# ibharvey/speq

Measured on AMD Instinct MI355X. Metric: k-mers scanned/sec (whole node) at k=21, 150 bp reads, higher is better.
Workload: dtype u32; 1 GPU; BASELINE config 2: 10 variants x 1 isolates x 50000 bp, 1000000 x 150 bp reads per GPU, k=21, global; k=21, reads_per_gpu=1000000, paired=False, mode=global, parallelism=dp1 (reads sharded, index replicated), collective=none (one GPU), gpus_visible=1, ranks_per_gpu=1, index_builder=gpu, fm_text_len=1000021

## Files before the change

### include/speq_scan.h

```cpp
#ifndef SPEQ_SCAN_H
#define SPEQ_SCAN_H

#include <stddef.h>
#include <stdint.h>

#ifdef __cplusplus
extern "C" {
#endif

#define SPEQ_ABI_VERSION 8

enum {
    SPEQ_OK = 0,
    SPEQ_E_ARG = -1,
    SPEQ_E_IO = -2,
    SPEQ_E_DEVICE = -3,
    SPEQ_E_GROUPS = -4,
    SPEQ_E_NOMEM = -5,
    SPEQ_E_RETRY = -6
};

enum { SPEQ_MODE_GLOBAL = 0, SPEQ_MODE_LOCAL = 1 };

typedef struct speq_index speq_index;
// ... 5 lines not shown
    uint32_t pair_steps;
    uint32_t label_table;
    uint32_t gpu_build;
    int32_t device;
    uint32_t triple_steps;
} speq_build_opts;

typedef struct {
    uint32_t k;
    uint32_t phred_cutoff;
    uint32_t paired;
    uint32_t mode;
} speq_scan_params;

#define SPEQ_COUNTS_LEN(G) ((size_t)(G) + 2u)

const char* speq_last_error(void);
int speq_abi_version(void);
int speq_device_count(void);

int speq_index_build(const char* seq, const uint64_t* rec_offsets, uint32_t n_records,
                     const int32_t* group_of_rec, uint32_t n_group_entries, uint32_t n_groups,
                     const speq_build_opts* opts, speq_index** out);
int speq_index_save(const speq_index* idx, const char* path, const void* user_header, uint64_t header_len);
int speq_index_load(const char* path, speq_index** out, void** user_header, uint64_t* header_len);
int speq_index_read_header(const char* path, void** user_header, uint64_t* header_len);
void speq_index_free(speq_index* idx);
void speq_free(void* p);

typedef struct {
    uint64_t n;
    uint32_t n_texts;
    uint32_t n_records;
    uint32_t n_groups;
    uint32_t prefix_q;
    uint32_t pair_steps;
    uint32_t label_table;
    uint64_t n_runs;
    uint64_t device_bytes;
    uint32_t triple_steps;
} speq_index_info;
int speq_index_get_info(const speq_index* idx, speq_index_info* info);

int speq_index_array(const speq_index* idx, const char* name, const void** ptr, uint64_t* bytes);

int speq_device_warmup(int device, uint32_t streams);
int speq_device_open(const speq_index* idx, int device, speq_device_index** out);
int speq_device_close(speq_device_index* d);

int speq_scan_reads_device(speq_device_index* d, const uint8_t* d_seq, const uint8_t* d_qual,
                           const uint64_t* d_offsets, uint64_t n_reads, const speq_scan_params* params,
                           uint64_t* d_counts, double* d_weights, void* stream);

#define SPEQ_AX_STATS_N 40
int speq_scan_reads_device_stats(speq_device_index* d, const uint8_t* d_seq, const uint8_t* d_qual,
                                 const uint64_t* d_offsets, uint64_t n_reads, const speq_scan_params* params,
                                 uint64_t* d_counts, double* d_weights, uint64_t* stats);

int speq_scan_reads(speq_device_index* d, const uint8_t* seq, const uint8_t* qual, const uint64_t* offsets,
                    uint64_t n_reads, const speq_scan_params* params, uint64_t* counts, double* weights);

#define SPEQ_REPORT_MAX_K 1024
typedef struct {
    uint32_t passing;
    uint32_t unique;
    uint32_t shared;
    uint32_t first_group;
} speq_read_report;
#define SPEQ_SET_WORDS(G) (((size_t)(G) + 63u) / 64u)
int speq_report_reads_device(speq_device_index* d, const uint8_t* d_seq, const uint8_t* d_qual,
                             const uint64_t* d_offsets, uint64_t n_reads, const speq_scan_params* params,
                             speq_read_report* d_reports, uint64_t* d_sets, void* stream);
int speq_report_reads(speq_device_index* d, const uint8_t* seq, const uint8_t* qual, const uint64_t* offsets,
                      uint64_t n_reads, const speq_scan_params* params, speq_read_report* reports, uint64_t* sets);
#define SPEQ_MARKER_BINS 8
typedef struct {
    uint64_t markers, observed, hits, max_depth, depth_hist[SPEQ_MARKER_BINS];
} speq_marker_cov;
typedef struct speq_markers speq_markers;
int speq_markers_create(speq_device_index* d, const speq_scan_params* params, speq_markers** out);
int speq_markers_add_reads_device(speq_markers* m, const uint8_t* d_seq, const uint8_t* d_qual,
                                  const uint64_t* d_offsets, uint64_t n_reads, void* stream);
int speq_markers_add_reads(speq_markers* m, const uint8_t* seq, const uint8_t* qual, const uint64_t* offsets,
                           uint64_t n_reads);
int speq_markers_finalize(speq_markers* m, speq_marker_cov* out);
int speq_markers_list(speq_markers* m, uint64_t* n_markers, uint32_t* lo, uint32_t* group, uint32_t* depth);
void speq_markers_free(speq_markers* m);

#define SPEQ_BOOTSTRAP_MAX_REPLICATES 1024
typedef struct speq_bootstrap speq_bootstrap;
int speq_bootstrap_create(speq_device_index* d, const speq_scan_params* params, uint32_t replicates, uint64_t seed,
                          speq_bootstrap** out);
int speq_bootstrap_add_reads_device(speq_bootstrap* b, const uint8_t* d_seq, const uint8_t* d_qual,
                                    const uint64_t* d_offsets, uint64_t n_reads, uint64_t first_unit, void* stream);
int speq_bootstrap_add_reads(speq_bootstrap* b, const uint8_t* seq, const uint8_t* qual, const uint64_t* offsets,
                             uint64_t n_reads, uint64_t first_unit);
int speq_bootstrap_finalize(speq_bootstrap* b, uint64_t* counts, double* weights);
int speq_bootstrap_info(const speq_bootstrap* b, uint32_t* replicates, uint32_t* lds_path, uint64_t* units_added);
void speq_bootstrap_free(speq_bootstrap* b);
uint32_t speq_bootstrap_weight(uint64_t seed, uint64_t unit, uint32_t replicate);
typedef struct { double estimate, mean, se, lo, hi; uint64_t used; } speq_bootstrap_ci;
int speq_bootstrap_summary(const uint64_t* counts, const double* weights, uint32_t replicates, uint32_t n_groups,
                           const uint64_t* u_ref, const uint64_t* tot_ref, double unique_scale, double level,
                           speq_bootstrap_ci* out );
int speq_bootstrap_summary_percent(const double* percent, const double* estimate, const uint8_t* used_mask,
                                   uint32_t replicates, uint32_t n_groups, double level,
                                   speq_bootstrap_ci* out );
// ... 168 lines not shown
```

### speq_amd/api.py

```python
from __future__ import annotations

import ctypes as C
from dataclasses import dataclass
from typing import Optional, Sequence

import numpy as np

from ._lib import (MARKER_BINS, SPEQ_MODE_GLOBAL, SPEQ_MODE_LOCAL, BootstrapCI, BuildOpts, IndexInfo,
                   DedupStatsRecord, ScanParams, Slot, SpeqError, StreamStats, check, lib)

__all__ = ["FmIndex", "DeviceIndex", "Node", "Pipeline", "ScanResult", "ReadReport", "Markers", "MarkerCoverage", "Bootstrap",
           "Dedup", "DedupStats", "dedup_fingerprint", "bootstrap_summary", "bootstrap_summary_percent", "em_rows_step", "em_rows_refine", "Groupings", "EmHistogram", "Comm", "file_to_map", "unique_to_percent",
           "em_refine", "pack_records", "SpeqError", "SPEQ_MODE_GLOBAL", "SPEQ_MODE_LOCAL"]


def _u64p(a: np.ndarray):
    return a.ctypes.data_as(C.POINTER(C.c_uint64))


def pack_records(records: Sequence[bytes | str]) -> tuple[bytes, np.ndarray]:
    bs = [r.encode() if isinstance(r, str) else bytes(r) for r in records]
    off = np.zeros(len(bs) + 1, dtype=np.uint64)
    if bs:
        off[1:] = np.cumsum([len(b) for b in bs], dtype=np.uint64)
# ... 259 lines not shown
                  phred_cutoff: int = 30, paired: bool = False, local: bool = False, first_unit: int = 0):
        b = Bootstrap(self, k, replicates, seed, phred_cutoff, paired, local)
        try:
            b.add(seq, qual, offsets, first_unit)
            return b.finalize()
        finally:
            b.close()

    def bootstrap_fastq(self, path1: str, path2: Optional[str] = None, k: int = 21, replicates: int = 200,
                        seed: int = 1, phred_cutoff: int = 30, local: bool = False, threads: int = 4):
        G = self.n_groups
        counts = np.zeros((replicates + 1, G + 2), dtype=np.uint64)
        w = np.zeros((replicates + 1, G), dtype=np.float64) if local else None
        p = ScanParams(k, phred_cutoff, int(path2 is not None), SPEQ_MODE_LOCAL if local else SPEQ_MODE_GLOBAL)
        check(lib().speq_bootstrap_fastq(self._h, path1.encode(), path2.encode() if path2 else None, C.byref(p),
                                         replicates, seed, threads, _u64p(counts),
                                         w.ctypes.data_as(C.POINTER(C.c_double)) if w is not None else None, None))
        return counts, w

    def bootstrap_em_fastq(self, em: "EmHistogram", path1: str, path2: Optional[str] = None, k: int = 21,
                           replicates: int = 200, seed: int = 1, phred_cutoff: int = 30, local: bool = False,
                           threads: int = 4):
        G = self.n_groups
        counts = np.zeros((replicates + 1, G + 2), dtype=np.uint64)
        w = np.zeros((replicates + 1, G), dtype=np.float64) if local else None
        mult = np.zeros((replicates + 1, em.n_rows()), dtype=np.uint64)
        missed = C.c_uint64()
        p = ScanParams(k, phred_cutoff, int(path2 is not None), SPEQ_MODE_LOCAL if local else SPEQ_MODE_GLOBAL)
        check(lib().speq_bootstrap_em_fastq(self._h, em._h, path1.encode(), path2.encode() if path2 else None,
                                            C.byref(p), replicates, seed, threads, _u64p(counts),
                                            w.ctypes.data_as(C.POINTER(C.c_double)) if w is not None else None,
                                            _u64p(mult), C.byref(missed), None))
        return counts, w, mult, missed.value

    def dedup_fastq(self, path1: str, path2: Optional[str] = None, k: int = 21, phred_cutoff: int = 30,
                    local: bool = False, threads: int = 4, em: Optional["EmHistogram"] = None):
        G = self.n_groups
        counts = np.zeros(G + 2, dtype=np.uint64)
        w = np.zeros(G, dtype=np.float64) if local else None
        p = ScanParams(k, phred_cutoff, int(path2 is not None), SPEQ_MODE_LOCAL if local else SPEQ_MODE_GLOBAL)
        r = DedupStatsRecord()
        check(lib().speq_dedup_fastq(self._h, em._h if em is not None else None, path1.encode(),
                                     path2.encode() if path2 else None, C.byref(p), threads, C.byref(r),
                                     _u64p(counts), w.ctypes.data_as(C.POINTER(C.c_double)) if w is not None else None,
                                     None))
        return DedupStats.from_record(r), ScanResult(int(counts[0]), int(counts[1]), counts[2:].copy(), w)

    AX_STATS_KEYS = ("wave_iters", "lookup_lanes", "run_lanes", "lookup_waves", "run_waves", "run_windows",
                     "deferred", "filter_pass", "p2_probes", "p2_verify", "chunks", "segments", "qual_bytes",
                     "run_tallied", "run_granules", "refills", "busy_1_4", "busy_5_16", "busy_17_32", "busy_33_64",
                     "cyc_refill", "cyc_lookup", "cyc_run", "cyc_phase2", "cyc_total", "p2_passes",
                     "cyc_p2_filter", "p2_rounds", "cyc_ref_pre", "cyc_ref_stage", "cyc_wave_max", "waves",
                     "cyc_gen0", "cyc_gen1", "cyc_gen2", "cyc_gen3", "cyc_gen4",
                     "sproof_probes", "sproof_windows", "sproof_partial")

    def scan_device_stats(self, d_seq: int, d_qual: int, d_offsets: int, n_reads: int, k: int, d_counts: int,
                          d_weights: int = 0, phred_cutoff: int = 30, paired: bool = False,
                          local: bool = False) -> dict:
        p = ScanParams(k, phred_cutoff, int(paired), SPEQ_MODE_LOCAL if local else SPEQ_MODE_GLOBAL)
        st = np.zeros(len(self.AX_STATS_KEYS), dtype=np.uint64)
        check(lib().speq_scan_reads_device_stats(self._h, d_seq, d_qual, d_offsets, n_reads, C.byref(p), d_counts,
                                                 d_weights or None, _u64p(st)))
        return {key: int(v) for key, v in zip(self.AX_STATS_KEYS, st)}

    def scan_fastq(self, path1: str, path2: Optional[str] = None, k: int = 21, phred_cutoff: int = 30,
                   local: bool = False, threads: int = 4, em: Optional["EmHistogram"] = None):
        G = self.n_groups
        counts = np.zeros(G + 2, dtype=np.uint64)
        w = np.zeros(G, dtype=np.float64) if local else None
        p = ScanParams(k, phred_cutoff, int(path2 is not None), SPEQ_MODE_LOCAL if local else SPEQ_MODE_GLOBAL)
        st = StreamStats()
        check(lib().speq_scan_fastq(self._h, path1.encode(), path2.encode() if path2 else None, C.byref(p),
                                    em._h if em is not None else None, threads, _u64p(counts),
                                    w.ctypes.data_as(C.POINTER(C.c_double)) if w is not None else None,
                                    C.byref(st)))
        stats = {"records": st.records, "bases": st.bases, "batches": st.batches, "seconds": st.seconds}
        return ScanResult(int(counts[0]), int(counts[1]), counts[2:].copy(), w), stats

    def scan_fastq_shard(self, path1: str, path2: Optional[str], k: int, shard: int, n_shards: int, cut: int = 0,
                         phred_cutoff: int = 30, local: bool = False, threads: int = 4,
                         em: Optional["EmHistogram"] = None):
        G = self.n_groups
        counts = np.zeros(G + 2, dtype=np.uint64)
        w = np.zeros(G, dtype=np.float64) if local else None
        p = ScanParams(k, phred_cutoff, int(path2 is not None), SPEQ_MODE_LOCAL if local else SPEQ_MODE_GLOBAL)
        st = StreamStats()
        check(lib().speq_scan_fastq_shard(self._h, em._h if em is not None else None, path1.encode(),
                                          path2.encode() if path2 else None, C.byref(p), threads, shard, n_shards,
                                          cut, _u64p(counts),
                                          w.ctypes.data_as(C.POINTER(C.c_double)) if w is not None else None,
                                          C.byref(st)))
        stats = {"records": st.records, "bases": st.bases, "batches": st.batches, "seconds": st.seconds}
        return ScanResult(int(counts[0]), int(counts[1]), counts[2:].copy(), w), stats

    def count_unique_kmers_per_group_shard(self, k: int, shard: int, n_shards: int):
        G = self.n_groups
        u = np.zeros(G, dtype=np.uint64)
        t = np.zeros(G, dtype=np.uint64)
        check(lib().speq_ref_unique_shard(self._h, k, shard, n_shards, _u64p(u), _u64p(t)))
        return u, t

    def count_unique_kmers_per_group(self, k: int) -> tuple[np.ndarray, np.ndarray]:
        G = self.n_groups
        u = np.zeros(G, dtype=np.uint64)
        t = np.zeros(G, dtype=np.uint64)
        check(lib().speq_ref_unique(self._h, k, _u64p(u), _u64p(t)))
        return u, t
# ... 572 lines not shown
```

### speq_amd/csrc/ax_common.hpp

```cpp
#pragma once
#include <hip/hip_runtime.h>

#include <cstdint>

#include "scan_device.hpp"
#include "speq_scan.h"

namespace speq_dev {
struct AxView {
    const u32x4* gran;
    const uint32_t* mlo;
    const uint32_t* mhi;
    const unsigned long long* atab;
    const unsigned long long* filt;
    unsigned long long* stats;
    uint64_t nb;
    uint64_t nf;
    uint64_t n;
    uint64_t gran_bytes;
    uint64_t nmf;
    uint32_t mf_off;
    uint32_t m;
    uint32_t mtiles;
    uint32_t s_off;
    uint32_t s_bytes;
    uint32_t G;
};
}

namespace {

using namespace speq_dev;

constexpr uint32_t AX_MAX_K = 128;
constexpr uint32_t AX_CAP = 192;
constexpr uint32_t AX_STREAM = AX_CAP + 16;
constexpr uint32_t AX_CHUNKS = AX_STREAM / 16;
constexpr uint32_t AX_CMP = 160;
constexpr uint32_t AX_CMPW = AX_CMP / 32;
constexpr uint32_t AX_NGR = AX_CMPW + 1;
constexpr uint32_t AX_CHK = 3;
constexpr uint32_t AX_VWW = 4;
#ifndef SPEQ_AX_DEF_LOCAL
#define SPEQ_AX_DEF_LOCAL 416
#endif
#ifndef SPEQ_AX_DEF_GLOBAL
#define SPEQ_AX_DEF_GLOBAL 864
#endif
template <int MODE>
constexpr uint32_t ax_def() {
    return MODE == KM_LOCAL ? SPEQ_AX_DEF_LOCAL : SPEQ_AX_DEF_GLOBAL;
}
static_assert(SPEQ_AX_DEF_GLOBAL % 4 == 0 && SPEQ_AX_DEF_LOCAL % 4 == 0, "u64 counters after the deferred list");
constexpr uint32_t AX_F = 4;
constexpr uint32_t AX_EMPTY = 0xFFFFFFFFu;
constexpr uint16_t AX_VOID = 0xFFFFu;
constexpr unsigned long long AX_SLOT_EMPTY = ~0ull;
constexpr uint32_t AX_OOB = 0xFFFFFFF0u;
constexpr uint32_t AX_FILTER_BITS = 16;
constexpr uint32_t AX_MP = 4;
constexpr uint32_t AX_MAX_G = 0xFFFFu;
typedef unsigned int u32x2 __attribute__((ext_vector_type(2)));

enum : uint32_t { AX_OWN = 0, AX_MULTI = 1, AX_SENT = 2, AX_END = 3 };

static_assert(AX_STREAM % 16 == 0, "chunks of 16 bases");
static_assert(AX_CAP < 1024, "deferred entries hold the window in 10 bits");
static_assert(AX_CMP % 32 == 0 && AX_CMP <= AX_CAP && 64 * AX_CHK >= AX_CMP, "run geometry");

enum : uint32_t {
    AXS_WAVE_ITERS = 0,
    AXS_LOOKUP_LANES,
    AXS_RUN_LANES,
    AXS_LOOKUP_WAVES,
    AXS_RUN_WAVES,
    AXS_RUN_WINDOWS,
    AXS_DEFERRED,
    AXS_FILTER_PASS,
    AXS_P2_PROBES,
    AXS_P2_VERIFY,
    AXS_CHUNKS,
    AXS_SEGMENTS,
    AXS_QBYTES,
    AXS_RUN_TALLIED,
    AXS_RUN_GRANULES,
    AXS_REFILLS,
    AXS_BUSY_1_4,
    AXS_BUSY_5_16,
    AXS_BUSY_17_32,
    AXS_BUSY_33_64,
    AXS_CYC_REFILL,
    AXS_CYC_LOOKUP,
    AXS_CYC_RUN,
    AXS_CYC_P2,
    AXS_CYC_TOTAL,
    AXS_P2_PASSES,
    AXS_CYC_P2_FILTER,
    AXS_P2_ROUNDS,
    AXS_CYC_REF_PRE,
    AXS_CYC_REF_STAGE,
    AXS_CYC_WAVE_MAX,
    AXS_WAVES,
    AXS_CYC_GEN0,
    AXS_CYC_GEN1,
    AXS_CYC_GEN2,
    AXS_CYC_GEN3,
    AXS_CYC_GEN4,
    AXS_SPROOF_PROBES,
    AXS_SPROOF_WINDOWS,
    AXS_SPROOF_PARTIAL,
    AXS_N
};
static_assert(AXS_N == SPEQ_AX_STATS_N, "speq_scan.h SPEQ_AX_STATS_N");

__host__ __device__ __forceinline__ uint64_t ax_fmix(uint64_t x) {
    x ^= x >> 33;
    x *= 0xFF51AFD7ED558CCDull;
    x ^= x >> 33;
    x *= 0xC4CEB9FE1A85EC53ull;
    x ^= x >> 33;
    return x;
}

template <int NW>
__device__ __forceinline__ uint64_t ax_hash(const uint64_t (&w)[NW], uint32_t k) {
    uint64_t h = 0x9E3779B97F4A7C15ull * (uint64_t)(k + 1u);
#pragma unroll
    for (int i = 0; i < NW; ++i) {
        if (32u * (uint32_t)i < k) {
            const uint32_t rem = k - 32u * (uint32_t)i;
            uint64_t x = w[i];
            if (rem < 32u) x &= (1ull << (2u * rem)) - 1ull;
            h = ax_fmix(h ^ x);
        }
    }
    return h;
}
__host__ __device__ __forceinline__ uint32_t ax_bucket(uint64_t h, uint64_t nb) {
    return (uint32_t)(((h >> 32) * nb) >> 32);
}
__host__ __device__ __forceinline__ uint32_t ax_fp(uint64_t h) { return (uint32_t)h & 0xFFFFu; }
__host__ __device__ __forceinline__ uint32_t ax_fword(uint64_t h, uint64_t nf) {
    return (uint32_t)((((h >> 24) & 0xFFFFFFFFull) * nf) >> 32);
}
__host__ __device__ __forceinline__ uint64_t ax_fbits(uint64_t h) {
    return (1ull << (h & 63u)) | (1ull << ((h >> 6) & 63u)) | (1ull << ((h >> 12) & 63u));
}

__device__ __forceinline__ uint64_t funnel(uint64_t lo, uint64_t hi, uint32_t sh) {
    return sh == 0u ? lo : ((lo >> sh) | (hi << (64u - sh)));
}
__device__ __forceinline__ uint64_t u64of(uint32_t lo, uint32_t hi) { return (uint64_t)lo | ((uint64_t)hi << 32); }

__device__ __forceinline__ uint32_t zero_bytes(uint32_t v) {
    return ~(((v & 0x7F7F7F7Fu) + 0x7F7F7F7Fu) | v) & 0x80808080u;
}
__device__ __forceinline__ uint32_t flags4(uint32_t m) {
    uint32_t y = m >> 7;
    y |= y >> 7;
    y |= y >> 14;
    return y & 0xFu;
}

// ... 21 lines not shown
            pp = fm == (uint32_t)t ? pos[t] : pp;
            gg = fm == (uint32_t)t ? fg[t] : gg;
        }
        p = pp;
        g = gg & 0xFFFFu;
        slot = fm;
        return 1u;
    }
    return fe < 8u ? 0u : 2u;
}

__device__ __forceinline__ bool ax_probe(const AxView& A, const __amdgpu_buffer_rsrc_t& rs_atab, uint32_t fp,
                                         uint32_t& b, uint32_t& s, uint32_t& p, uint32_t& g, bool active,
                                         uint32_t& probes) {
    bool found = false, pending = active;
    while (__ballot(pending) != 0) {
        const uint32_t boff = pending ? b * 64u : AX_OOB;
        const u32x4 v0 = __builtin_amdgcn_raw_buffer_load_b128(rs_atab, boff, 0, 0);
        const u32x4 v1 = __builtin_amdgcn_raw_buffer_load_b128(rs_atab, boff + 16u, 0, 0);
        const u32x4 v2 = __builtin_amdgcn_raw_buffer_load_b128(rs_atab, boff + 32u, 0, 0);
        const u32x4 v3 = __builtin_amdgcn_raw_buffer_load_b128(rs_atab, boff + 48u, 0, 0);
        if (pending) {
            ++probes;
            uint32_t slot = 0;
            const uint32_t r = ax_resolve(v0, v1, v2, v3, fp, s, slot, p, g);
            if (r == 1u) {
                s = slot;
                found = true;
                pending = false;
            } else if (r == 0u) {
                pending = false;
            } else {
                b = (b + 1u == (uint32_t)A.nb) ? 0u : b + 1u;
                s = 0;
            }
        }
    }
    return found;
}

constexpr uint32_t AX_FONE = 76u, AX_FTAB = AX_FONE + 1u;
static_assert(8u * (AX_FTAB + QLUT_LEN) <= QTAB_BYTES && AX_FONE - 1u == 33u + 41u + 1u, "ftab + wtab in QTAB_BYTES");
#ifndef SPEQ_AX_WL
#define SPEQ_AX_WL 128
#endif
constexpr uint32_t AX_WL = SPEQ_AX_WL;
static_assert(AX_WL % 64u == 0 && AX_WL >= 64u && AX_WL <= 512u, "work list: 1-8 sub-batches of 64 blocks per round");
#ifndef SPEQ_AX_SU
#define SPEQ_AX_SU 3
#endif
#ifndef SPEQ_AX_SU_LOCAL
#define SPEQ_AX_SU_LOCAL 3
#endif
template <int MODE, bool PAIRED, int HW>
constexpr uint32_t ax_su() {
    return MODE == KM_LOCAL ? SPEQ_AX_SU_LOCAL
                            : ((HW == 3 || (PAIRED && HW == 2)) && SPEQ_AX_SU > 2 ? 2u : SPEQ_AX_SU);
}
template <int MODE>
constexpr uint32_t ax_ownb() {
    return 64u * (MODE == KM_LOCAL ? SPEQ_AX_SU_LOCAL : SPEQ_AX_SU);
}
template <int MODE>
constexpr uint32_t ax_wave_bytes() {
    static_assert(8u * AX_VWW >= 2u * AX_CHUNKS, "the bad-base bits of a staged piece live in its valid-window words");
    return 4u * AX_CHUNKS * 64u + 8u * AX_VWW * 64u + (MODE == KM_LOCAL ? 2u * AX_CHUNKS * 64u : 0u) +
           64u + 2u * ax_def<MODE>() + 24u + 8u * 64u + (MODE == KM_LOCAL ? 4u * AX_WL + 4u * 64u : 0u) +
           ax_ownb<MODE>();
}

#ifndef SPEQ_AX_WPB
#define SPEQ_AX_WPB 4
#endif
constexpr uint32_t AX_WPB = SPEQ_AX_WPB, AX_THREADS = 64 * SPEQ_AX_WPB;
#ifndef SPEQ_AX_MIN_WAVES
#define SPEQ_AX_MIN_WAVES 5
#endif
#ifndef SPEQ_AX_MIN_WAVES_LOCAL
#define SPEQ_AX_MIN_WAVES_LOCAL 4
#endif
#ifndef SPEQ_AX_REFILL
#define SPEQ_AX_REFILL 16
#endif
#ifndef SPEQ_AX_BLOCKED
#define SPEQ_AX_BLOCKED 16
#endif
#ifndef SPEQ_AX_SPEC_HW
#define SPEQ_AX_SPEC_HW 3
#endif
#ifndef SPEQ_AX_PRIO
#define SPEQ_AX_PRIO 1
#endif
#ifndef SPEQ_AX_PRIO_MIN
#define SPEQ_AX_PRIO_MIN 384u
#endif
#ifndef SPEQ_AX_MPROOF
#define SPEQ_AX_MPROOF 1
#endif
#ifndef SPEQ_AX_MTILES
#define SPEQ_AX_MTILES 1
#endif
#if !defined(SPEQ_AX_SPROOF)
#define SPEQ_AX_SPROOF 1
#endif
#ifndef SPEQ_AX_P2_MARGIN
#define SPEQ_AX_P2_MARGIN 256u
// ... 18 lines not shown
```

### speq_amd/csrc/ax_scan.hip

```cpp
#include <hip/hip_runtime.h>

#include <algorithm>
#include <chrono>
#include <climits>
#include <cstdint>
#include <cstdlib>
#include <cstring>
#include <mutex>
#include <stdexcept>
#include <type_traits>
#include <vector>

#include "device_index.hpp"
#include "fm_index.hpp"
#include "scan_device.hpp"
#include "scan_internal.hpp"
#include "speq_scan.h"
#include "ax_common.hpp"

namespace {

using namespace speq_dev;


// ... 262 lines not shown
    double* ftab = reinterpret_cast<double*>(smem + hist_bytes);
    double* wtab = ftab + AX_FTAB;
    const uint32_t qtab_bytes = MODE == KM_LOCAL ? QTAB_BYTES : 0u;
    constexpr uint32_t WAVE_BYTES = ax_wave_bytes<MODE>();
    unsigned char* wb = smem + hist_bytes + qtab_bytes + wid * WAVE_BYTES;
    uint32_t* codes = reinterpret_cast<uint32_t*>(wb);
    uint64_t* vw = reinterpret_cast<uint64_t*>(codes + AX_CHUNKS * 64u);
    uint16_t* bad16 = reinterpret_cast<uint16_t*>(vw);
    uint16_t* chg = reinterpret_cast<uint16_t*>(vw + AX_VWW * 64u);
    uint8_t* off0s = reinterpret_cast<uint8_t*>(chg + (MODE == KM_LOCAL ? AX_CHUNKS * 64u : 0u));
    uint16_t* defl = reinterpret_cast<uint16_t*>(off0s + 64);
    constexpr uint32_t AX_DEF = ax_def<MODE>();
    uint32_t* defn = reinterpret_cast<uint32_t*>(defl + AX_DEF);
    unsigned long long* wsum = reinterpret_cast<unsigned long long*>(defn + 2);
    int32_t* ambf = reinterpret_cast<int32_t*>(defn + 6);
    int32_t* ambd = ambf + 64;
    uint32_t* wl = reinterpret_cast<uint32_t*>(ambd + 64);
    uint32_t* wlm = wl + AX_WL;
    uint8_t* ownb = reinterpret_cast<uint8_t*>(MODE == KM_LOCAL ? wlm + 64 : wl);

    if (MODE == KM_LOCAL)
        for (uint32_t i = threadIdx.x; i < AX_FTAB; i += AX_THREADS) {
            const int q = (int)i - 33;
            ftab[i] = i == AX_FONE ? 1.0 : src.qlut[2 * (q < 0 ? 0 : (q > 41 ? 41 : q)) + 1];
            if (i < QLUT_LEN) {
                const double lut = src.qlut[2 * i], inv = src.qlut[2 * i + 1];
                double x = 1.0;
                for (uint32_t j = 0; j < k; ++j) x = div_rn(x, lut, inv);
                wtab[i] = x;
            }
        }
    if (LDS_HIST)
        for (uint32_t i = threadIdx.x; i < hist_words; i += AX_THREADS) hA[i] = 0ull;
    if (lane == 0) {
        defn[0] = defn[1] = 0u;
        wsum[0] = wsum[1] = 0ull;
    }
    __syncthreads();
    unsigned long long* gU = out_a + 2;

    const __amdgpu_buffer_rsrc_t rs_gran =
        __builtin_amdgcn_make_buffer_rsrc((void*)A.gran, (short)0, (int)(uint32_t)A.gran_bytes, 0x00020000);
    const __amdgpu_buffer_rsrc_t rs_atab = __builtin_amdgcn_make_buffer_rsrc(
        (void*)A.atab, (short)0,
        (int)(uint32_t)((SPEQ_AX_SPROOF && SP && A.s_bytes != 0u) ? A.s_off + A.s_bytes
                                                             : A.nb * 64u + (A.m != 0u ? A.nmf * 8u + 16u : 0u)),
        0x00020000);
    const __amdgpu_buffer_rsrc_t rs_filt =
        __builtin_amdgcn_make_buffer_rsrc((void*)A.filt, (short)0, (int)(uint32_t)(A.nf * 8u), 0x00020000);
    const uint64_t NWV = (uint64_t)gridDim.x * AX_WPB;
    const uint64_t gw = (uint64_t)blockIdx.x * AX_WPB + wid;
    const uint64_t nu = PAIRED ? src.n_units / 2 : src.n_units;
    const uint32_t segw = AX_CAP - k + 1u;
    const uint32_t qt = 33u + src.cutoff;
    const uint32_t qt4 = (qt > 0x7Fu ? 0x7Fu : qt) * 0x01010101u;
    const uint32_t allbad = src.cutoff >= 41u ? 0x80808080u : 0u;

    uint32_t s_iter = 0, s_lk = 0, s_rn = 0, s_lkw = 0, s_rnw = 0, s_rwin = 0, s_def = 0, s_fp = 0, s_p2 = 0,
             s_p2v = 0, s_ch = 0, s_seg = 0, s_qb = 0, s_tal = 0, s_rg = 0, s_spl = 0, s_b4 = 0, s_b16 = 0, s_b32 = 0,
             s_b64 = 0, s_p2n = 0, s_p2r = 0, s_spp = 0, s_spw = 0, s_spt = 0;
    uint64_t c_ref = 0, c_lk = 0, c_rn = 0, c_p2 = 0, c_p2f = 0, c_rpre = 0, c_rstg = 0, c_t0 = STATS ? clock64() : 0ull, c_s = 0;

    auto add_count = [&](uint32_t g, uint32_t cnt, double wsum) {
        if (LDS_HIST) {
            atomicAdd(&hA[g], (unsigned long long)cnt);
            if (MODE == KM_LOCAL && wsum != 0.0) atomicAdd(&hW[g], wsum);
        } else {
            atomicAdd(&gU[g], (unsigned long long)cnt);
            if (MODE == KM_LOCAL && wsum != 0.0) atomicAdd(&out_w[g], wsum);
        }
    };
    auto add_weight = [&](uint32_t g, double w) {
        if (LDS_HIST) atomicAdd(&hW[g], w);
        else atomicAdd(&out_w[g], w);
    };
    auto slot64 = [&](uint32_t o, uint32_t pos) -> uint64_t {
        const uint32_t d = pos >> 4, sh = 2u * (pos & 15u);
        const uint32_t w0 = d < AX_CHUNKS ? codes[d * 64u + o] : 0u;
        const uint32_t w1 = d + 1u < AX_CHUNKS ? codes[(d + 1u) * 64u + o] : 0u;
        const uint32_t w2 = d + 2u < AX_CHUNKS ? codes[(d + 2u) * 64u + o] : 0u;
        return u64of(alignbit(w1, w0, sh), alignbit(w2, w1, sh));
    };
    auto read_words = [&](uint32_t o, uint32_t pos, uint64_t(&w)[HW]) {
        if (HW <= 2) {
#pragma unroll
            for (int i = 0; i < HW; ++i) w[i] = slot64(o, pos + 32u * (uint32_t)i);
            return;
        }
        const uint32_t d = pos >> 4, sh = 2u * (pos & 15u);
        uint32_t c[2 * HW + 1];
#pragma unroll
        for (int i = 0; i <= 2 * HW; ++i) c[i] = d + (uint32_t)i < AX_CHUNKS ? codes[(d + (uint32_t)i) * 64u + o] : 0u;
#pragma unroll
        for (int i = 0; i < HW; ++i) w[i] = u64of(alignbit(c[2 * i + 1], c[2 * i], sh), alignbit(c[2 * i + 2], c[2 * i + 1], sh));
    };
    auto vbits = [&](uint32_t o, uint32_t b) -> uint64_t {
        const uint32_t w0 = b >> 6, s6 = b & 63u;
        const uint64_t lo = w0 < AX_VWW ? vw[w0 * 64u + o] : 0ull;
        const uint64_t hi = w0 + 1u < AX_VWW ? vw[(w0 + 1u) * 64u + o] : 0ull;
        return funnel(lo, hi, s6);
    };
    auto next_valid = [&](uint32_t o, uint32_t j, uint32_t end) -> uint32_t {
        for (uint32_t b = j; b < end; b += 64u) {
            const uint64_t v = vbits(o, b);
            if (v) return min(b + (uint32_t)__builtin_ctzll(v), end);
        }
        return end;
    };
    auto fac = [&](uint32_t x) -> double { return ftab[min(x & 0xFFu, AX_FONE - 1u)]; };
    auto weight8 = [&](uint64_t qo, uint32_t mask) -> double {
        const uintptr_t ad = reinterpret_cast<uintptr_t>(src.qual + qo);
        const uint32_t* wp = reinterpret_cast<const uint32_t*>(ad & ~(uintptr_t)3);
        const uint32_t sh = (uint32_t)ad & 3u;
// ... 102 lines not shown
    uint32_t gt = 0;
    int32_t last_mm = -1;
    uint32_t pb = 0, ps = 0;
    bool resume = false;
    bool run_phase = true;
    constexpr bool SPEC = HW >= SPEQ_AX_SPEC_HW && !EM && MODE == KM_LOCAL;
    constexpr uint32_t AX_PS_SPEC = 16u, AX_PS_FRESH = 17u;
    constexpr bool SPROOF = SPEQ_AX_SPROOF != 0 && SP;
    constexpr uint32_t AX_PS_SFRESH = 18u;
    constexpr bool MTILES = SPEQ_AX_MTILES && !SPEC;
    uint32_t sp = 0;
    auto defer_except = [&](uint32_t lo, uint32_t hi, uint64_t x0, uint64_t x1)
                            __attribute__((always_inline)) -> bool {
        if (hi + 1u <= lo) return true;
        const uint32_t span = hi + 1u - lo;
        uint64_t dm0 = vbits(lane, lo) & ~x0, dm1 = span > 64u ? (vbits(lane, lo + 64u) & ~x1) : 0ull;
        dm0 &= span >= 64u ? ~0ull : ((1ull << span) - 1ull);
        if (span > 64u) dm1 &= span - 64u >= 64u ? ~0ull : ((1ull << (span - 64u)) - 1ull);
        const uint32_t cnt = (uint32_t)__popcll(dm0) + (uint32_t)__popcll(dm1);
        if (cnt == 0u) return true;
        const uint32_t slot0 = atomicAdd(&defn[0], cnt);
        if (slot0 + cnt > AX_DEF) {
            for (uint32_t sl = slot0; sl < AX_DEF && sl < slot0 + cnt; ++sl) defl[sl] = AX_VOID;
            st = 3u;
            hasdef = true;
            return false;
        }
        uint32_t sl = slot0;
        for (uint64_t t = dm0; t; t &= t - 1) defl[sl++] = (uint16_t)(lane | ((lo + (uint32_t)__builtin_ctzll(t)) << 6));
        for (uint64_t t = dm1; t; t &= t - 1)
            defl[sl++] = (uint16_t)(lane | ((lo + 64u + (uint32_t)__builtin_ctzll(t)) << 6));
        hasdef = true;
        if (STATS) s_def += cnt;
        return true;
    };
    auto defer_range = [&](uint32_t lo, uint32_t hi) __attribute__((always_inline)) -> bool {
        return defer_except(lo, hi, 0ull, 0ull);
    };

    auto start_read_at = [&](uint64_t r, uint64_t b, uint64_t e) {
        rd = (uint32_t)r;
        rb = b;
        L = (uint32_t)(e - b);
        W = L >= k ? L - k + 1 : 0;
        nseg = W ? (uint32_t)((W + segw - 1) / segw) : 1u;
        seg = 0;
    };
    auto start_read = [&](uint64_t r) { start_read_at(r, src.off[r], src.off[r + 1]); };
    uint32_t L2m = 0;

    constexpr uint32_t SU = ax_su<MODE, PAIRED, HW>();
    static_assert(64u * SU <= ax_ownb<MODE>(), "owner map of one batch");
    static_assert(AX_CHUNKS < 16, "chunk counts in four bits");
    uint32_t stg_tot = 0;
    uint32_t stg_ocarry = 0;
    uint32_t stg_qcarry = 0;
    uint32_t stg_pre = 0, stg_nch = 0;
    auto stage_issue = [&](uint32_t c0, uint4(&sv)[SU], uint4(&qv)[SU], uint32_t(&dst)[SU]) {
#pragma unroll
        for (uint32_t u = 0; u < SU; ++u) ownb[64u * u + lane] = 0;
        if (stg_nch != 0u && stg_pre >= c0 && stg_pre < c0 + 64u * SU) ownb[stg_pre - c0] = (uint8_t)(lane + 1u);
        wave_sync();
        uint32_t mk[SU];
#pragma unroll
        for (uint32_t u = 0; u < SU; ++u) mk[u] = ownb[64u * u + lane];
#pragma unroll
        for (uint32_t u = 0; u < SU; ++u) {
            const uint32_t c = min(c0 + 64u * u + lane, stg_tot - 1u);
            uint32_t m = mk[u];
            m = max(m, (uint32_t)__builtin_amdgcn_update_dpp(0, (int)m, 0x111, 0xF, 0xF, false));
            m = max(m, (uint32_t)__builtin_amdgcn_update_dpp(0, (int)m, 0x112, 0xF, 0xF, false));
            m = max(m, (uint32_t)__builtin_amdgcn_update_dpp(0, (int)m, 0x114, 0xF, 0xF, false));
            m = max(m, (uint32_t)__builtin_amdgcn_update_dpp(0, (int)m, 0x118, 0xF, 0xF, false));
            m = max(m, (uint32_t)__builtin_amdgcn_update_dpp(0, (int)m, 0x142, 0xA, 0xF, false));
            m = max(m, (uint32_t)__builtin_amdgcn_update_dpp(0, (int)m, 0x143, 0xC, 0xF, false));
            m = max(m, stg_ocarry);
            stg_ocarry = (uint32_t)__builtin_amdgcn_readlane((int)m, 63);
            const uint32_t o = m - 1u;
            const uint32_t ci = c - (uint32_t)__shfl((int)stg_pre, (int)o);
            dst[u] = ci * 64u + o;
            const uint64_t go = ((uint64_t)__shfl((long long)ta, (int)o) & ~15ull) + 16ull * ci;
            sv[u] = *reinterpret_cast<const uint4*>(src.seq + go);
            qv[u] = *reinterpret_cast<const uint4*>(src.qual + go);
        }
    };
    auto stage_decode = [&](uint32_t c0, const uint4(&sv)[SU], const uint4(&qv)[SU], const uint32_t(&dst)[SU]) {
#pragma unroll
        for (uint32_t u = 0; u < SU; ++u) {
            const uint32_t c = c0 + 64u * u + lane;
            const uint32_t sd[4] = {sv[u].x, sv[u].y, sv[u].z, sv[u].w};
            const uint32_t qd[4] = {qv[u].x, qv[u].y, qv[u].z, qv[u].w};
            uint32_t cw = 0, bad = 0, chb = 0;
            uint32_t qprev = 0;
            if (MODE == KM_LOCAL) {
                const uint32_t up = (uint32_t)__builtin_amdgcn_update_dpp(0, (int)qv[u].w, 0x138, 0xF, 0xF, false);
                qprev = lane == 0 ? stg_qcarry : up;
                stg_qcarry = __builtin_amdgcn_readlane(qv[u].w, 63);
            }
#pragma unroll
            for (int i = 0; i < 4; ++i) {
                const uint32_t x = sd[i] | 0x20202020u;
                const uint32_t c4 = ((x >> 1) ^ (x >> 2)) & 0x03030303u;
                cw |= ((c4 | (c4 >> 6) | (c4 >> 12) | (c4 >> 18)) & 0xFFu) << (8 * i);
                const uint32_t canon = __builtin_amdgcn_perm(0u, 0x74676361u, c4);
                const uint32_t okb = zero_bytes(x ^ canon) | zero_bytes(x ^ 0x75757575u);
                const uint32_t y = qd[i];
                const uint32_t badq = (((0x80808080u | qt4) - (y & 0x7F7F7F7Fu)) & ~y & 0x80808080u) | allbad;
                bad |= flags4((~okb & 0x80808080u) | badq) << (4 * i);
                if (MODE == KM_LOCAL) {
                    const uint32_t prev = (y << 8) | (qprev >> 24);
                    chb |= flags4(~zero_bytes(y ^ prev) & 0x80808080u) << (4 * i);
                    qprev = y;
                }
            }
            if (c < stg_tot) {
                const uint32_t ci = dst[u] >> 6, o = dst[u] & 63u;
                codes[dst[u]] = cw;
                bad16[((ci >> 2) * 64u + o) * 4u + (ci & 3u)] = (uint16_t)bad;
                if (MODE == KM_LOCAL) chg[dst[u]] = (uint16_t)chb;
            }
        }
    };
    auto finish_piece = [&](uint32_t nch) {
        uint32_t ok[8];
        {
            const uint32_t* vw32 = reinterpret_cast<const uint32_t*>(vw);
            const uint32_t nb = 16u * nch;
#pragma unroll
            for (uint32_t d = 0; d < 8u; ++d) {
                const uint32_t b0 = 32u * d;
                uint32_t v = vw32[((d >> 1) * 64u + lane) * 2u + (d & 1u)];
                v |= nb <= b0 ? ~0u : (nb < b0 + 32u ? ~0u << (nb - b0) : 0u);
                ok[d] = ~v;
            }
        }
        for (uint32_t len = 1u; len < k;) {
            const uint32_t sft = min(len, k - len);
            const uint32_t dw = sft >> 5, bs = sft & 31u;
            if (dw == 0u) {
#pragma unroll
                for (uint32_t d = 0; d < 8u; ++d) ok[d] &= alignbit(d + 1u < 8u ? ok[d + 1] : 0u, ok[d], bs);
            } else if (dw == 1u) {
#pragma unroll
                for (uint32_t d = 0; d < 8u; ++d)
                    ok[d] &= alignbit(d + 2u < 8u ? ok[d + 2] : 0u, d + 1u < 8u ? ok[d + 1] : 0u, bs);
            } else {
#pragma unroll
                for (uint32_t d = 0; d < 8u; ++d) ok[d] &= d + 2u < 8u ? ok[d + 2] : 0u;
            }
            len += sft;
        }
        {
            uint32_t* vw32 = reinterpret_cast<uint32_t*>(vw);
            uint32_t tc = 0;
#pragma unroll
            for (uint32_t d = 0; d < 2u * AX_VWW; ++d) {
                uint32_t v = alignbit(d + 1u < 8u ? ok[d + 1] : 0u, ok[d], off0);
                const uint32_t bit0 = 32u * d;
                v = wend <= bit0 ? 0u : (wend < bit0 + 32u ? v & ((1u << (wend - bit0)) - 1u) : v);
                tc += (uint32_t)__popc(v);
                vw32[((d >> 1) * 64u + lane) * 2u + (d & 1u)] = v;
            }
            if (tc) atomicAdd(&wsum[0], (unsigned long long)tc);
        }
        j = 0;
        if (SPEC) sp = 0;
        st = wend > 0 ? 0u : 2u;
// ... 168 lines not shown
                        if (PAIRED) {
                            const uint64_t r0 = 2 * newu, o0 = src.off[r0], o1 = src.off[r0 + 1], o2 = src.off[r0 + 2];
                            start_read_at(r0, o0, o1);
                            L2m = (uint32_t)(o2 - o1);
                        } else {
                            start_read(newu);
                        }
                        stg = true;
                    }
                } else if (seg + 1u < nseg) {
                    ++seg;
                    stg = true;
                } else {
                    mate = 1;
                    start_read_at(rd + 1, rb + L, rb + L + L2m);
                    stg = true;
                }
            }
            const uint64_t s = (uint64_t)seg * segw;
            const uint32_t sb = stg && W ? (uint32_t)(L - s < AX_CAP ? L - s : AX_CAP) : 0u;
            const uint32_t nwend = stg && W ? (uint32_t)(W - s < segw ? W - s : segw) : 0u;
            const uint64_t a = rb + s;
            const uint64_t a16 = a & ~15ull;
            const uint32_t noff0 = (uint32_t)(a - a16);
            const uint32_t nch = sb ? (noff0 + sb + 15u) / 16u : 0u;
            if (stg) {
                last_piece = seg + 1u >= nseg && (!PAIRED || mate == 1u);
                wend = nwend;
                off0 = noff0;
                ta = a;
                off0s[lane] = (uint8_t)noff0;
                if (STATS) {
                    s_ch += nch;
                    s_seg += 1u;
                }
            }
            uint32_t pre = 0, nch_tot = 0;
#pragma unroll
            for (uint32_t bb = 0; bb < 4; ++bb) {
                const unsigned long long m = __ballot((nch >> bb) & 1u);
                pre += lanes_below(m) << bb;
                nch_tot += (uint32_t)__popcll(m) << bb;
            }
            stg_pre = pre;
            stg_nch = stg ? nch : 0u;
            stg_tot = nch_tot;
            stg_ocarry = 0;
            stg_qcarry = 0;
            uint64_t c_b = 0;
            if (STATS) {
                c_b = clock64();
                c_rpre += c_b - c_s;
            }
            for (uint32_t c0 = 0; c0 < nch_tot; c0 += 64u * SU) {
                uint4 sv[SU], qv[SU];
                uint32_t dst[SU];
                stage_issue(c0, sv, qv, dst);
                stage_decode(c0, sv, qv, dst);
            }
            wave_sync();
            if (STATS) c_rstg += clock64() - c_b;
            if (stg) finish_piece(nch);
            if (STATS) c_ref += clock64() - c_s;
            continue;
        }
        if (busy == 0) continue;

        const unsigned long long busy1 = __ballot(st != 2u);
        if (busy1 == 0) continue;
        if (STATS && lane == 0) {
            const uint32_t nb = (uint32_t)__popcll(busy1);
            s_b4 += nb <= 4u ? 1u : 0u;
            s_b16 += (nb > 4u && nb <= 16u) ? 1u : 0u;
            s_b32 += (nb > 16u && nb <= 32u) ? 1u : 0u;
            s_b64 += nb > 32u ? 1u : 0u;
        }
        const bool want_lk = __ballot(st == 0u || st >= 4u) != 0, want_rn = __ballot(st == 1u) != 0;
        run_phase = run_phase ? !want_lk : want_rn;
        constexpr bool SPEC_RW = HW == 1 && !PAIRED;
        uint64_t ra[HW];
        if (!run_phase && st == 0u) {
            const uint32_t j0 = j;
            if (SPEC_RW) read_words(lane, off0 + j0, ra);
            j = next_valid(lane, j0, wend);
            if (SPEC && sp != 0u && j >= wend && defer_range(sp, min(sp + k - 2u, wend - 1u)))
                sp = 0;
            if (j >= wend && st == 0u) st = 2u;
            else if (SPEC_RW && j != j0) read_words(lane, off0 + j, ra);
        }
        const bool lk = st == 0u && !run_phase, rn = st == 1u && run_phase;
        if (STATS) {
            s_iter += lane == 0 ? 1u : 0u;
            s_lkw += (lane == 0 && !run_phase) ? 1u : 0u;
            s_rnw += (lane == 0 && run_phase) ? 1u : 0u;
            s_lk += lk ? 1u : 0u;
            s_rn += rn ? 1u : 0u;
        }
        if (!run_phase) {
            if (!SPEC_RW) read_words(lane, off0 + j, ra);
            const uint64_t h = ax_hash<HW>(ra, k);
            const uint32_t fp = ax_fp(h);
            if (lk && !resume) {
                pb = ax_bucket(h, A.nb);
                ps = 0;
            }
            const uint32_t boff = lk ? pb * 64u : AX_OOB;
            uint32_t o0 = boff, o1 = lk ? boff + 16u : AX_OOB, o2 = lk ? boff + 32u : AX_OOB,
                     o3 = lk ? boff + 48u : AX_OOB;
            const bool sprobe = SPROOF && st == 7u;
            if (SPROOF && sprobe) o0 = A.s_off + ((p + k - 1u) >> 5) * 4u;
            const bool mk = SPEQ_AX_MPROOF && st >= 4u && !sprobe;
            const uint32_t km = k - A.m;
// ... 431 lines not shown
                    while (nzb != 0u && pre < r0 + AX_WL) {
                        const uint32_t blk = (uint32_t)__builtin_ctz(nzb);
                        nzb &= nzb - 1u;
                        const uint32_t c = blk >> 2;
                        const uint32_t oc = c == 0u ? ownc[0] : (c == 1u ? ownc[1] : (c == 2u ? ownc[2] : (c == 3u ? ownc[3] : ownc[4])));
                        wl[pre - r0] = lane | (blk << 6) | (((oc >> (8u * (blk & 3u))) & 0xFFu) << 11);
                        ++pre;
                    }
                    wave_sync();
                    const uint32_t tot = min(all - r0, AX_WL);
                    for (uint32_t b0 = 0; b0 < tot; b0 += 64u) {
                        const uint32_t en = wl[min(b0 + lane, AX_WL - 1u)];
                        const uint64_t qo = (uint64_t)__shfl((long long)ta, (int)(en & 63u));
                        if (b0 + lane < tot) {
                            const uint32_t o = en & 63u, meta = wlm[o];
                            const uint32_t jb = (meta >> 16) + 8u * ((en >> 6) & 31u);
                            double s = 0.0;
                            if (k >= 8u) {
                                s = weight8(qo + jb, en >> 11);
                            } else {
                                const uint32_t so = (uint32_t)off0s[o];
                                for (uint32_t m = en >> 11; m; m &= m - 1u) {
                                    const uint32_t jj = jb + (uint32_t)__builtin_ctz(m);
                                    s += weight(qo + jj, chg_zero(o, so + jj + 1u, k - 1u));
                                }
                            }
                            add_weight(meta & 0xFFFFu, s);
                        }
                    }
                    wave_sync();
                }
            }
        }
        if (STATS) {
            if (run_phase) c_rn += clock64() - c_s;
            else c_lk += clock64() - c_s;
        }
    }
    const uint64_t c_tot = STATS ? clock64() - c_t0 : 0ull;
    if (has_unit && ad) atomicAdd(&wsum[1], 1ull);
    wave_sync();
    const unsigned long long tsum = wsum[0], asum = wsum[1];
    if (!LDS_HIST && lane == 0) {
        if (tsum) atomicAdd(&out_a[0], tsum);
        if (asum) atomicAdd(&out_a[1], asum);
    }
    if (STATS) {
        const uint64_t sv[AXS_N] = {s_iter, s_lk, s_rn, s_lkw, s_rnw, s_rwin, s_def, s_fp, s_p2, s_p2v, s_ch, s_seg,
                                    s_qb, s_tal, s_rg, s_spl, s_b4, s_b16, s_b32, s_b64,
                                    lane == 0 ? c_ref : 0ull, lane == 0 ? c_lk : 0ull, lane == 0 ? c_rn : 0ull,
                                    lane == 0 ? c_p2 : 0ull, lane == 0 ? c_tot : 0ull, s_p2n,
                                    lane == 0 ? c_p2f : 0ull, s_p2r, lane == 0 ? c_rpre : 0ull,
                                    lane == 0 ? c_rstg : 0ull, 0ull, lane == 0 ? 1ull : 0ull, 0ull, 0ull, 0ull, 0ull,
                                    0ull, s_spp, s_spw, s_spt};
#pragma unroll
        for (uint32_t i = 0; i < AXS_N; ++i)
            if (sv[i]) atomicAdd(&A.stats[i], (unsigned long long)sv[i]);
        if (lane == 0) {
            atomicMax(&A.stats[AXS_CYC_WAVE_MAX], (unsigned long long)c_tot);
            atomicAdd(&A.stats[AXS_CYC_GEN0 + min(blockIdx.x / 256u, 4u)], (unsigned long long)c_tot);
        }
    }
    if (LDS_HIST) {
        __syncthreads();
        for (uint32_t i = threadIdx.x; i < G + 2u; i += AX_THREADS) {
            unsigned long long x = 0;
            if (i < 2u) {
#pragma unroll
                for (uint32_t w = 0; w < AX_WPB; ++w)
                    x += reinterpret_cast<const unsigned long long*>(
                        smem + hist_bytes + qtab_bytes + w * WAVE_BYTES +
                        (reinterpret_cast<const unsigned char*>(wsum) - wb))[i];
            } else {
                x = hA[i - 2u];
            }
            if (x) atomicAdd(&out_a[i], x);
        }
        for (uint32_t g = threadIdx.x; g < (MODE == KM_LOCAL ? G : 0u); g += AX_THREADS) {
            if (MODE == KM_LOCAL) {
                const double y = hW[g];
                if (y != 0.0) atomicAdd(&out_w[g], y);
            }
        }
    }
}

template <int MODE, bool PAIRED, bool LDS, bool EM, int HW, bool STATS, bool SP>
void ax_launch_one(const AxView& A, const UnitSrc& src, uint32_t grid, size_t lds, hipStream_t st,
                  unsigned long long* a, double* w, uint32_t n_cus) {
    if (lds > 64 * 1024)
        HIP_OK(hipFuncSetAttribute(reinterpret_cast<const void*>(&k_scan_ax<MODE, PAIRED, LDS, EM, HW, STATS, SP>),
                                   hipFuncAttributeMaxDynamicSharedMemorySize, 160 * 1024));
    static std::mutex mu;
    static size_t cached_lds = 0;
    static int cached_blocks = 0;
    int per_cu = 0;
    {
        std::lock_guard<std::mutex> lk(mu);
        if (cached_lds != lds || cached_blocks == 0) {
            int nb = 0;
            HIP_OK(hipOccupancyMaxActiveBlocksPerMultiprocessor(
                &nb, reinterpret_cast<const void*>(&k_scan_ax<MODE, PAIRED, LDS, EM, HW, STATS, SP>), AX_THREADS, lds));
            cached_lds = lds;
            cached_blocks = std::max(nb, 1);
        }
        per_cu = cached_blocks;
    }
// ... 263 lines not shown
```

Baseline: 1022 billion k-mers/s.

## Size final stage batch to remaining slots and streamline chunk decode

The refill staging loop now processes whole SU-wide batches and then a smaller N-wide tail batch, so it no longer issues loads and decodes for empty 64-chunk slots. The per-chunk base/quality decode moves into a shared helper that uses udot4 and a nonzero-byte trick to build the code words and bad flags with fewer instructions. A sched_barrier separates load issue from decode. This adds extra template instantiations (more code size, possible register pressure) and a new stats counter.

```diff
diff --git a/include/speq_scan.h b/include/speq_scan.h
--- a/include/speq_scan.h
+++ b/include/speq_scan.h
@@ -81,7 +81,7 @@
                            const uint64_t* d_offsets, uint64_t n_reads, const speq_scan_params* params,
                            uint64_t* d_counts, double* d_weights, void* stream);
 
-#define SPEQ_AX_STATS_N 40
+#define SPEQ_AX_STATS_N 41
 int speq_scan_reads_device_stats(speq_device_index* d, const uint8_t* d_seq, const uint8_t* d_qual,
                                  const uint64_t* d_offsets, uint64_t n_reads, const speq_scan_params* params,
                                  uint64_t* d_counts, double* d_weights, uint64_t* stats);
diff --git a/speq_amd/api.py b/speq_amd/api.py
--- a/speq_amd/api.py
+++ b/speq_amd/api.py
@@ -335,7 +335,7 @@
                      "cyc_refill", "cyc_lookup", "cyc_run", "cyc_phase2", "cyc_total", "p2_passes",
                      "cyc_p2_filter", "p2_rounds", "cyc_ref_pre", "cyc_ref_stage", "cyc_wave_max", "waves",
                      "cyc_gen0", "cyc_gen1", "cyc_gen2", "cyc_gen3", "cyc_gen4",
-                     "sproof_probes", "sproof_windows", "sproof_partial")
+                     "sproof_probes", "sproof_windows", "sproof_partial", "stage_slots")
 
     def scan_device_stats(self, d_seq: int, d_qual: int, d_offsets: int, n_reads: int, k: int, d_counts: int,
                           d_weights: int = 0, phred_cutoff: int = 30, paired: bool = False,
diff --git a/speq_amd/csrc/ax_common.hpp b/speq_amd/csrc/ax_common.hpp
--- a/speq_amd/csrc/ax_common.hpp
+++ b/speq_amd/csrc/ax_common.hpp
@@ -3,6 +3,7 @@
 
 #include <cstdint>
 
+#include "ax_decode.hpp"
 #include "scan_device.hpp"
 #include "speq_scan.h"
 
@@ -109,6 +110,7 @@
     AXS_SPROOF_PROBES,
     AXS_SPROOF_WINDOWS,
     AXS_SPROOF_PARTIAL,
+    AXS_STAGE_SLOTS,
     AXS_N
 };
 static_assert(AXS_N == SPEQ_AX_STATS_N, "speq_scan.h SPEQ_AX_STATS_N");
@@ -236,6 +238,9 @@
 #ifndef SPEQ_AX_SU_LOCAL
 #define SPEQ_AX_SU_LOCAL 3
 #endif
+#if !defined(SPEQ_AX_STAGE_SKIP)
+#define SPEQ_AX_STAGE_SKIP 1
+#endif
 template <int MODE, bool PAIRED, int HW>
 constexpr uint32_t ax_su() {
     return MODE == KM_LOCAL ? SPEQ_AX_SU_LOCAL
diff --git a/speq_amd/csrc/ax_decode.hpp b/speq_amd/csrc/ax_decode.hpp
--- /dev/null
+++ b/speq_amd/csrc/ax_decode.hpp
@@ -0,0 +1,74 @@
+#pragma once
+#include <cstdint>
+
+#if defined(__HIPCC__)
+#define AXD_FN __host__ __device__ inline __attribute__((always_inline))
+#else
+#define AXD_FN inline
+#endif
+
+namespace speq_dev {
+
+AXD_FN uint32_t axd_perm4(uint32_t tab, uint32_t sel) {
+#if defined(__HIP_DEVICE_COMPILE__)
+    return __builtin_amdgcn_perm(0u, tab, sel);
+#else
+    uint32_t r = 0;
+    for (int j = 0; j < 4; ++j) r |= ((tab >> (8u * ((sel >> (8 * j)) & 3u))) & 0xFFu) << (8 * j);
+    return r;
+#endif
+}
+AXD_FN uint32_t axd_udot4(uint32_t a, uint32_t b, uint32_t acc) {
+#if defined(__HIP_DEVICE_COMPILE__)
+    return __builtin_amdgcn_udot4(a, b, acc, false);
+#else
+    for (int j = 0; j < 4; ++j) acc += ((a >> (8 * j)) & 0xFFu) * ((b >> (8 * j)) & 0xFFu);
+    return acc;
+#endif
+}
+AXD_FN uint32_t axd_nonzero_top(uint32_t v) { return ((v & 0x7F7F7F7Fu) + 0x7F7F7F7Fu) | v; }
+
+AXD_FN uint32_t axd_qt4(uint32_t cutoff) {
+    const uint32_t qt = cutoff > 0x7Fu - 33u ? 0x7Fu : 33u + cutoff;
+    return qt * 0x01010101u;
+}
+AXD_FN uint32_t axd_allbad(uint32_t cutoff) { return cutoff >= 41u ? 0x80808080u : 0u; }
+
+template <bool LOCAL>
+AXD_FN void ax_decode_chunk(const uint32_t (&sd)[4], const uint32_t (&qd)[4], uint32_t qt4, uint32_t allbad,
+                            uint32_t qprev, uint32_t& cw, uint32_t& bad, uint32_t& chb) {
+    uint32_t c = 0, bl = 0, bh = 0, hl = 0, hh = 0;
+    uint32_t qp = qprev << 24;
+#if defined(__clang__)
+#pragma unroll
+#endif
+    for (int i = 0; i < 4; ++i) {
+        const uint32_t x = sd[i] | 0x20202020u;
+        const uint32_t c4 = ((x >> 1) ^ (x >> 2)) & 0x03030303u;
+        c |= axd_udot4(c4, 0x40100401u, 0u) << (8 * i);
+        const uint32_t canon = axd_perm4(0x74676361u, c4);
+        const uint32_t x2 = x & ~((x >> 4) & 0x01010101u);
+        const uint32_t nzb = axd_nonzero_top(x2 ^ canon);
+        const uint32_t y = qd[i];
+        const uint32_t badq = (((0x80808080u | qt4) - (y & 0x7F7F7F7Fu)) & ~y) | allbad;
+        const uint32_t f = ((nzb | badq) >> 7) & 0x01010101u;
+        if (i == 0) bl = axd_udot4(f, 0x08040201u, 0u);
+        if (i == 1) bl = axd_udot4(f, 0x80402010u, bl);
+        if (i == 2) bh = axd_udot4(f, 0x08040201u, 0u);
+        if (i == 3) bh = axd_udot4(f, 0x80402010u, bh);
+        if (LOCAL) {
+            const uint32_t prev = (y << 8) | (qp >> 24);
+            const uint32_t g = (axd_nonzero_top(y ^ prev) >> 7) & 0x01010101u;
+            if (i == 0) hl = axd_udot4(g, 0x08040201u, 0u);
+            if (i == 1) hl = axd_udot4(g, 0x80402010u, hl);
+            if (i == 2) hh = axd_udot4(g, 0x08040201u, 0u);
+            if (i == 3) hh = axd_udot4(g, 0x80402010u, hh);
+            qp = y;
+        }
+    }
+    cw = c;
+    bad = bl | (bh << 8);
+    chb = hl | (hh << 8);
+}
+
+}
diff --git a/speq_amd/csrc/ax_scan.hip b/speq_amd/csrc/ax_scan.hip
--- a/speq_amd/csrc/ax_scan.hip
+++ b/speq_amd/csrc/ax_scan.hip
@@ -338,13 +338,11 @@
     const uint64_t gw = (uint64_t)blockIdx.x * AX_WPB + wid;
     const uint64_t nu = PAIRED ? src.n_units / 2 : src.n_units;
     const uint32_t segw = AX_CAP - k + 1u;
-    const uint32_t qt = 33u + src.cutoff;
-    const uint32_t qt4 = (qt > 0x7Fu ? 0x7Fu : qt) * 0x01010101u;
-    const uint32_t allbad = src.cutoff >= 41u ? 0x80808080u : 0u;
+    const uint32_t qt4 = axd_qt4(src.cutoff), allbad = axd_allbad(src.cutoff);
 
     uint32_t s_iter = 0, s_lk = 0, s_rn = 0, s_lkw = 0, s_rnw = 0, s_rwin = 0, s_def = 0, s_fp = 0, s_p2 = 0,
              s_p2v = 0, s_ch = 0, s_seg = 0, s_qb = 0, s_tal = 0, s_rg = 0, s_spl = 0, s_b4 = 0, s_b16 = 0, s_b32 = 0,
-             s_b64 = 0, s_p2n = 0, s_p2r = 0, s_spp = 0, s_spw = 0, s_spt = 0;
+             s_b64 = 0, s_p2n = 0, s_p2r = 0, s_spp = 0, s_spw = 0, s_spt = 0, s_slots = 0;
     uint64_t c_ref = 0, c_lk = 0, c_rn = 0, c_p2 = 0, c_p2f = 0, c_rpre = 0, c_rstg = 0, c_t0 = STATS ? clock64() : 0ull, c_s = 0;
 
     auto add_count = [&](uint32_t g, uint32_t cnt, double wsum) {
@@ -553,20 +551,24 @@
     constexpr uint32_t SU = ax_su<MODE, PAIRED, HW>();
     static_assert(64u * SU <= ax_ownb<MODE>(), "owner map of one batch");
     static_assert(AX_CHUNKS < 16, "chunk counts in four bits");
+    static_assert(SU >= 1u && SU <= 4u, "stage_batch is instantiated for 1 .. 4 stream instructions");
     uint32_t stg_tot = 0;
     uint32_t stg_ocarry = 0;
     uint32_t stg_qcarry = 0;
     uint32_t stg_pre = 0, stg_nch = 0;
-    auto stage_issue = [&](uint32_t c0, uint4(&sv)[SU], uint4(&qv)[SU], uint32_t(&dst)[SU]) {
-#pragma unroll
-        for (uint32_t u = 0; u < SU; ++u) ownb[64u * u + lane] = 0;
-        if (stg_nch != 0u && stg_pre >= c0 && stg_pre < c0 + 64u * SU) ownb[stg_pre - c0] = (uint8_t)(lane + 1u);
+    auto stage_batch = [&](auto n_const, uint32_t c0) __attribute__((always_inline)) {
+        constexpr uint32_t N = decltype(n_const)::value;
+        uint4 sv[N], qv[N];
+        uint32_t dst[N];
+#pragma unroll
+        for (uint32_t u = 0; u < N; ++u) ownb[64u * u + lane] = 0;
+        if (stg_nch != 0u && stg_pre >= c0 && stg_pre < c0 + 64u * N) ownb[stg_pre - c0] = (uint8_t)(lane + 1u);
         wave_sync();
-        uint32_t mk[SU];
-#pragma unroll
-        for (uint32_t u = 0; u < SU; ++u) mk[u] = ownb[64u * u + lane];
-#pragma unroll
-        for (uint32_t u = 0; u < SU; ++u) {
+        uint32_t mk[N];
+#pragma unroll
+        for (uint32_t u = 0; u < N; ++u) mk[u] = ownb[64u * u + lane];
+#pragma unroll
+        for (uint32_t u = 0; u < N; ++u) {
             const uint32_t c = min(c0 + 64u * u + lane, stg_tot - 1u);
             uint32_t m = mk[u];
             m = max(m, (uint32_t)__builtin_amdgcn_update_dpp(0, (int)m, 0x111, 0xF, 0xF, false));
@@ -584,10 +586,9 @@
             sv[u] = *reinterpret_cast<const uint4*>(src.seq + go);
             qv[u] = *reinterpret_cast<const uint4*>(src.qual + go);
         }
-    };
-    auto stage_decode = [&](uint32_t c0, const uint4(&sv)[SU], const uint4(&qv)[SU], const uint32_t(&dst)[SU]) {
-#pragma unroll
-        for (uint32_t u = 0; u < SU; ++u) {
+        __builtin_amdgcn_sched_barrier(0);
+#pragma unroll
+        for (uint32_t u = 0; u < N; ++u) {
             const uint32_t c = c0 + 64u * u + lane;
             const uint32_t sd[4] = {sv[u].x, sv[u].y, sv[u].z, sv[u].w};
             const uint32_t qd[4] = {qv[u].x, qv[u].y, qv[u].z, qv[u].w};
@@ -595,25 +596,10 @@
             uint32_t qprev = 0;
             if (MODE == KM_LOCAL) {
                 const uint32_t up = (uint32_t)__builtin_amdgcn_update_dpp(0, (int)qv[u].w, 0x138, 0xF, 0xF, false);
-                qprev = lane == 0 ? stg_qcarry : up;
+                qprev = (lane == 0 ? stg_qcarry : up) >> 24;
                 stg_qcarry = __builtin_amdgcn_readlane(qv[u].w, 63);
             }
-#pragma unroll
-            for (int i = 0; i < 4; ++i) {
-                const uint32_t x = sd[i] | 0x20202020u;
-                const uint32_t c4 = ((x >> 1) ^ (x >> 2)) & 0x03030303u;
-                cw |= ((c4 | (c4 >> 6) | (c4 >> 12) | (c4 >> 18)) & 0xFFu) << (8 * i);
-                const uint32_t canon = __builtin_amdgcn_perm(0u, 0x74676361u, c4);
-                const uint32_t okb = zero_bytes(x ^ canon) | zero_bytes(x ^ 0x75757575u);
-                const uint32_t y = qd[i];
-                const uint32_t badq = (((0x80808080u | qt4) - (y & 0x7F7F7F7Fu)) & ~y & 0x80808080u) | allbad;
-                bad |= flags4((~okb & 0x80808080u) | badq) << (4 * i);
-                if (MODE == KM_LOCAL) {
-                    const uint32_t prev = (y << 8) | (qprev >> 24);
-                    chb |= flags4(~zero_bytes(y ^ prev) & 0x80808080u) << (4 * i);
-                    qprev = y;
-                }
-            }
+            ax_decode_chunk<MODE == KM_LOCAL>(sd, qd, qt4, allbad, qprev, cw, bad, chb);
             if (c < stg_tot) {
                 const uint32_t ci = dst[u] >> 6, o = dst[u] & 63u;
                 codes[dst[u]] = cw;
@@ -888,12 +874,15 @@
                 c_b = clock64();
                 c_rpre += c_b - c_s;
             }
-            for (uint32_t c0 = 0; c0 < nch_tot; c0 += 64u * SU) {
-                uint4 sv[SU], qv[SU];
-                uint32_t dst[SU];
-                stage_issue(c0, sv, qv, dst);
-                stage_decode(c0, sv, qv, dst);
-            }
+            const uint32_t slots = (nch_tot + 63u) / 64u;
+            const uint32_t full = SPEQ_AX_STAGE_SKIP ? slots / SU : (slots + SU - 1u) / SU;
+            for (uint32_t b = 0; b < full; ++b) stage_batch(std::integral_constant<uint32_t, SU>{}, 64u * SU * b);
+            const uint32_t c1 = 64u * SU * full;
+            const uint32_t ns = SPEQ_AX_STAGE_SKIP ? slots % SU : 0u;
+            if (SU > 1u && ns == 1u) stage_batch(std::integral_constant<uint32_t, 1u>{}, c1);
+            if (SU > 2u && ns == 2u) stage_batch(std::integral_constant<uint32_t, (SU > 2u ? 2u : 1u)>{}, c1);
+            if (SU > 3u && ns == 3u) stage_batch(std::integral_constant<uint32_t, (SU > 3u ? 3u : 1u)>{}, c1);
+            if (STATS) s_slots += lane == 0 ? SU * full + ns : 0u;
             wave_sync();
             if (STATS) c_rstg += clock64() - c_b;
             if (stg) finish_piece(nch);
@@ -1431,7 +1420,7 @@
                                     lane == 0 ? c_p2 : 0ull, lane == 0 ? c_tot : 0ull, s_p2n,
                                     lane == 0 ? c_p2f : 0ull, s_p2r, lane == 0 ? c_rpre : 0ull,
                                     lane == 0 ? c_rstg : 0ull, 0ull, lane == 0 ? 1ull : 0ull, 0ull, 0ull, 0ull, 0ull,
-                                    0ull, s_spp, s_spw, s_spt};
+                                    0ull, s_spp, s_spw, s_spt, s_slots};
 #pragma unroll
         for (uint32_t i = 0; i < AXS_N; ++i)
             if (sv[i]) atomicAdd(&A.stats[i], (unsigned long long)sv[i]);
```

After: 1092 billion k-mers/s (median of 6 runs). 1.07x the previous value.
